# quickwit-oss/quickwit

Hardware: AMD Instinct MI355X
Metric: leaf_search_docs_per_sec (higher is better)
Workload: dtype u32+f32; 1 GPU; 3term_bm25_or_100000000; query=body:w00009 OR body:w00010 OR body:w00011, docs_per_gpu=100000000, splits_per_gpu=1, max_hits=10, parallelism=split-dp1

## Files before the change

include/quickwit_amd.h:

```cpp
#ifndef QUICKWIT_AMD_H
#define QUICKWIT_AMD_H

#include <stddef.h>
#include <stdint.h>

#ifdef __cplusplus
extern "C" {
#endif

typedef struct qw_ctx qw_ctx;

typedef struct qw_buf {
    uint8_t* data;
    size_t len;
} qw_buf;

enum qw_status {
    QW_OK = 0,
    QW_ERR_INVALID_ARGUMENT = -1,
    QW_ERR_INVALID_QUERY = -2,
    QW_ERR_NOT_FOUND = -3,
    QW_ERR_INTERNAL = -4,
    QW_ERR_NO_GPU = -5,
    QW_ERR_BAD_SPLIT = -6,
// ... 5 lines not shown

int32_t qw_ctx_add_split(qw_ctx* ctx, const char* split_id,
                         const uint8_t* data, size_t len);
int32_t qw_ctx_remove_split(qw_ctx* ctx, const char* split_id);

int32_t qw_leaf_search(qw_ctx* ctx, const uint8_t* leaf_search_request_pb,
                       size_t len, qw_buf* response_pb_out);

void qw_buf_free(qw_buf* buf);

int32_t qw_fetch_docs(qw_ctx* ctx, const uint8_t* fetch_docs_request_pb,
                      size_t len, qw_buf* response_pb_out);

int32_t qw_leaf_list_terms(qw_ctx* ctx, const uint8_t* leaf_list_terms_request_pb,
                           size_t len, qw_buf* response_pb_out);

int32_t qw_merge_leaf_responses(const uint8_t* search_request_pb,
                                size_t search_request_len,
                                const uint8_t** response_pbs,
                                const size_t* response_lens, size_t n,
                                qw_buf* merged_out);

int32_t qw_finalize_agg_to_json(const uint8_t* blob, size_t len,
                                const char* agg_request_json,
                                qw_buf* json_out);

int32_t qw_regex_match_terms(const char* regex, size_t regex_len,
                             const uint8_t* term_bytes,
                             const uint32_t* term_offsets, size_t num_terms,
                             uint64_t* match_bitmap_out);

int32_t qw_regex_table_stats(const char* regex, size_t regex_len,
                             uint64_t out[3]);

int32_t qw_regex_resolve(const char* regex, size_t regex_len,
                         int32_t tokenizer_lowercases, qw_buf* resolved_out);

const char* qw_last_error(const qw_ctx* ctx);


int32_t qw_kernel_stats(qw_ctx* ctx, const char* kernel_name,
                        double* total_ms, uint64_t* launches);
void qw_kernel_stats_reset(qw_ctx* ctx);
int32_t qw_ctx_device_sync(qw_ctx* ctx);

int32_t qw_ctx_memory_stats(qw_ctx* ctx, uint64_t* used_bytes,
                            uint64_t* budget_bytes, uint64_t* splits_bytes);

int32_t qw_absence_cache_stats(qw_ctx* ctx, uint64_t* hits, uint64_t* misses,
                               uint64_t* entries);

int32_t qw_topk_stats(qw_ctx* ctx, uint64_t out[4]);

const char* qw_version(void);

#ifdef __cplusplus
}
#endif

#endif
```

quickwit_amd/api.py:

```python
import ctypes
import json
import os

from . import proto

REPO_ROOT = os.path.dirname(os.path.dirname(os.path.abspath(__file__)))


class _Buf(ctypes.Structure):
    _fields_ = [("data", ctypes.POINTER(ctypes.c_uint8)), ("len", ctypes.c_size_t)]


def _bind(lib, syms):
    getattr(lib, syms["create"]).restype = ctypes.c_void_p
    getattr(lib, syms["add_split"]).argtypes = [
        ctypes.c_void_p, ctypes.c_char_p, ctypes.c_char_p, ctypes.c_size_t]
    getattr(lib, syms["leaf_search"]).argtypes = [
        ctypes.c_void_p, ctypes.c_char_p, ctypes.c_size_t, ctypes.POINTER(_Buf)]
    getattr(lib, syms["last_error"]).restype = ctypes.c_char_p
    getattr(lib, syms["last_error"]).argtypes = [ctypes.c_void_p]
    getattr(lib, syms["buf_free"]).argtypes = [ctypes.POINTER(_Buf)]


class _BaseSearcher:
# ... 106 lines not shown
    def leaf_list_terms(self, req: dict) -> dict:
        fn = self._lib.qw_leaf_list_terms
        fn.argtypes = [ctypes.c_void_p, ctypes.c_char_p, ctypes.c_size_t,
                       ctypes.POINTER(_Buf)]
        req_pb = proto.encode("LeafListTermsRequest", req)
        buf = _Buf()
        rc = fn(self._ctx, req_pb, len(req_pb), ctypes.byref(buf))
        if rc != 0:
            raise RuntimeError(f"leaf_list_terms failed ({rc}): {self._err()}")
        out = ctypes.string_at(buf.data, buf.len)
        self._lib.qw_buf_free(ctypes.byref(buf))
        return proto.decode("LeafListTermsResponse", out)

    def kernel_stats(self, name: str):
        fn = self._lib.qw_kernel_stats
        fn.argtypes = [ctypes.c_void_p, ctypes.c_char_p,
                       ctypes.POINTER(ctypes.c_double), ctypes.POINTER(ctypes.c_uint64)]
        ms = ctypes.c_double()
        n = ctypes.c_uint64()
        rc = fn(self._ctx, name.encode(), ctypes.byref(ms), ctypes.byref(n))
        if rc != 0:
            raise KeyError(name)
        return ms.value, n.value

    def kernel_stats_reset(self):
        self._lib.qw_kernel_stats_reset.argtypes = [ctypes.c_void_p]
        self._lib.qw_kernel_stats_reset(self._ctx)

    def memory_stats(self):
        fn = self._lib.qw_ctx_memory_stats
        fn.argtypes = [ctypes.c_void_p] + [ctypes.POINTER(ctypes.c_uint64)] * 3
        u, b, s = ctypes.c_uint64(), ctypes.c_uint64(), ctypes.c_uint64()
        rc = fn(self._ctx, ctypes.byref(u), ctypes.byref(b), ctypes.byref(s))
        if rc != 0:
            raise RuntimeError(f"memory_stats failed: {rc}")
        return u.value, b.value, s.value

    def absence_cache_stats(self):
        fn = self._lib.qw_absence_cache_stats
        fn.argtypes = [ctypes.c_void_p] + [ctypes.POINTER(ctypes.c_uint64)] * 3
        h, m, e = ctypes.c_uint64(), ctypes.c_uint64(), ctypes.c_uint64()
        rc = fn(self._ctx, ctypes.byref(h), ctypes.byref(m), ctypes.byref(e))
        if rc != 0:
            raise RuntimeError(f"absence_cache_stats failed: {rc}")
        return h.value, m.value, e.value

    def topk_stats(self):
        fn = self._lib.qw_topk_stats
        fn.argtypes = [ctypes.c_void_p, ctypes.POINTER(ctypes.c_uint64 * 4)]
        out = (ctypes.c_uint64 * 4)()
        rc = fn(self._ctx, ctypes.byref(out))
        if rc != 0:
            raise RuntimeError(f"topk_stats failed: {rc}")
        return tuple(out)

    def device_sync(self):
        self._lib.qw_ctx_device_sync.argtypes = [ctypes.c_void_p]
        rc = self._lib.qw_ctx_device_sync(self._ctx)
        if rc != 0:
            raise RuntimeError(f"device_sync failed: {self._err()}")


def _product_lib():
    path = os.environ.get("QW_PRODUCT_LIB") or os.path.join(
        REPO_ROOT, "libquickwit_amd.so")
    if not os.path.exists(path):
        raise FileNotFoundError(
            f"{path} not built — run __graft_entry__.build() first")
    lib = ctypes.CDLL(path)
    lib.qw_last_error.restype = ctypes.c_char_p
    lib.qw_last_error.argtypes = [ctypes.c_void_p]
    return lib


def regex_match_terms(regex: str | bytes, terms: list) -> list:
    lib = _product_lib()
    raw = [t.encode() if isinstance(t, str) else bytes(t) for t in terms]
    offsets = (ctypes.c_uint32 * (len(raw) + 1))()
    pos = 0
    for i, t in enumerate(raw):
        offsets[i] = pos
        pos += len(t)
    offsets[len(raw)] = pos
    packed = b"".join(raw)
    words = (ctypes.c_uint64 * max(1, (len(raw) + 63) // 64))()
    rx = regex.encode() if isinstance(regex, str) else bytes(regex)
    fn = lib.qw_regex_match_terms
    fn.argtypes = [ctypes.c_char_p, ctypes.c_size_t, ctypes.c_char_p,
                   ctypes.POINTER(ctypes.c_uint32), ctypes.c_size_t,
                   ctypes.POINTER(ctypes.c_uint64)]
    rc = fn(rx, len(rx), packed, offsets, len(raw), words)
    if rc != 0:
        msg = lib.qw_last_error(None)
        raise ValueError(msg.decode(errors="replace") if msg else f"rc={rc}")
    return [bool((words[i >> 6] >> (i & 63)) & 1) for i in range(len(raw))]


def regex_table_stats(regex: str | bytes) -> tuple:
    lib = _product_lib()
    fn = lib.qw_regex_table_stats
    fn.argtypes = [ctypes.c_char_p, ctypes.c_size_t,
                   ctypes.POINTER(ctypes.c_uint64 * 3)]
    rx = regex.encode() if isinstance(regex, str) else bytes(regex)
    out = (ctypes.c_uint64 * 3)()
    rc = fn(rx, len(rx), ctypes.byref(out))
    if rc != 0:
# ... 58 lines not shown
```

quickwit_amd/csrc/gpu_types.h:

```cpp
#pragma once
#include <cstdint>

namespace qw {

#ifndef QW_TILE_DOCS
#define QW_TILE_DOCS 8192
#endif
constexpr uint32_t TILE_DOCS = QW_TILE_DOCS;
constexpr uint32_t TILE_THREADS = 256;
constexpr uint32_t KTAB_LDS_MAX = 4;
constexpr uint32_t AGG_LDS_BUCKETS = 2048;
constexpr uint32_t TOPK_BINS = 4096;

enum TermRole : uint32_t { ROLE_SHOULD = 0, ROLE_MUST = 1, ROLE_MUST_NOT = 2 };

struct TermDev {
    uint32_t role;
    uint32_t grp;
    uint32_t n_blocks;
    uint64_t skip_off;
    uint64_t payload_off;
    uint64_t norms_off;
    float weight;
    uint32_t ktab_idx;
// ... 68 lines not shown
    uint32_t c_histo;
    uint32_t c_missing;
    double c_interval[4], c_offset[4];
    int64_t c_base[4];
    uint32_t p_si;
    uint64_t p_out;
    int32_t p_k_lo;
    uint32_t p_n_keys;
    uint64_t p_bound_off;
};

struct QueryDev {
    const uint8_t* split;
    const uint8_t* scratch;
    uint8_t* results;
    uint32_t num_docs;
    uint32_t n_tiles;
    uint32_t n_terms;
    uint32_t n_must;
    uint32_t n_must_not;
    uint32_t n_preds;
    uint32_t n_aggs;
    uint32_t msm;
    uint32_t scoring;
    uint32_t match_all;
    uint32_t collect_hits;
    uint32_t sort_asc;
    uint32_t wide_cand;
    uint32_t sort_src;
    uint32_t sort_width;
    uint64_t sort_values_off;
    uint64_t sort_nulls_off;
    uint32_t agg_fast;
    uint32_t agg_nt;
    uint32_t nt_decode;
    uint64_t bitmap_out;
    uint64_t terms_off;
    uint64_t preds_off;
    uint64_t aggs_off;
    uint64_t ktabs_off;
    uint32_t n_ktabs;
    uint32_t _pad_ktab;
    uint64_t norms_stage_off;
    uint64_t tile_counts_off;
    uint64_t cand_count_off;
    uint64_t cand_off;
    uint64_t cand_cap;
    uint64_t hist_off;
    uint32_t prune_k;
    uint32_t gates_off;
};

constexpr uint32_t TOPK_BOUND_OFF = 16;
constexpr uint32_t TOPK_PRUNE_MAX_K = 64;
inline uint32_t* cand_hdr_candidates(uint8_t* hdr) { return (uint32_t*)hdr; }
inline uint32_t* cand_hdr_survivors(uint8_t* hdr) { return (uint32_t*)hdr + 1; }
inline uint32_t* cand_hdr_cursor_band(uint8_t* hdr) { return (uint32_t*)hdr + 2; }

}
```

quickwit_amd/csrc/kernels.hip:

```cpp
#include <hip/hip_runtime.h>

#include "gpu_types.h"

namespace qw {

#pragma pack(push, 1)
struct SkipEntryDev {
    uint32_t first_doc;
    uint32_t last_doc;
    uint32_t word_off;
    uint8_t id_bits;
    uint8_t tf_bits;
    uint16_t count;
};
#pragma pack(pop)

__device__ __forceinline__ uint32_t lane_id() { return threadIdx.x & 63u; }

__device__ __forceinline__ uint64_t extract_bits(const uint32_t* base, uint64_t bitpos,
                                                 uint32_t w) {
    uint64_t word = bitpos >> 5;
    uint32_t sh = uint32_t(bitpos & 31);
    uint64_t v = (uint64_t(base[word]) | (uint64_t(base[word + 1]) << 32)) >> sh;
    return v & ((1ull << w) - 1ull);
// ... 1073 lines not shown
                                               uint32_t* hist) {
    __shared__ uint32_t lh[TOPK_BINS];
    for (uint32_t i = threadIdx.x; i < TOPK_BINS; i += bdim) lh[i] = 0;
    __syncthreads();
    uint32_t n = *n_ptr;
    uint32_t shift = 64 - prefix_bits - 12;
    uint32_t last_bin = 0xFFFFFFFFu, acc = 0;
    for (uint32_t i = blockIdx.x * bdim + threadIdx.x; i < n;
         i += gridDim.x * bdim) {
        uint64_t k = cand[RW * i];
        if (prefix_bits && (k >> (64 - prefix_bits)) != prefix) continue;
        uint32_t b = uint32_t(k >> shift) & (TOPK_BINS - 1);
        if (b == last_bin) ++acc;
        else {
            if (acc) atomicAdd(&lh[last_bin], acc);
            last_bin = b;
            acc = 1;
        }
    }
    if (acc) atomicAdd(&lh[last_bin], acc);
    __syncthreads();
    for (uint32_t i = threadIdx.x; i < TOPK_BINS; i += bdim)
        if (lh[i]) atomicAdd(&hist[i], lh[i]);
}

template <uint32_t RW>
__device__ __forceinline__ void cand_compact_body(uint32_t bdim,
                                                  const uint64_t* cand, uint32_t n,
                                                  uint64_t floor_key,
                                                  uint64_t ceil_key, uint64_t* out,
                                                  uint32_t* out_count,
                                                  uint32_t cap) {
    for (uint32_t i = blockIdx.x * bdim + threadIdx.x; i < n;
         i += gridDim.x * bdim) {
        uint64_t k = cand[RW * i];
        bool take = k >= floor_key && k <= ceil_key;
        uint64_t mask = __ballot(take);
        uint32_t nw = __popcll(mask);
        if (!nw) continue;
        uint32_t leader = __ffsll((unsigned long long)mask) - 1;
        uint32_t base;
        if (lane_id() == leader) base = atomicAdd(out_count, nw);
        base = __shfl(base, leader, 64);
        if (take) {
            uint32_t off = base + __popcll(mask & ((1ull << lane_id()) - 1ull));
            if (off < cap) {
                out[RW * off] = k;
                if (RW == 2) out[2 * off + 1] = cand[2 * i + 1];
            }
        }
    }
}

extern "C" __global__ void k_cand_hist(const uint64_t* cand, const uint32_t* n_ptr,
                                       uint64_t prefix, uint32_t prefix_bits,
                                       uint32_t* hist) {
    cand_hist_body<1>(blockDim.x, cand, n_ptr, prefix, prefix_bits, hist);
}
extern "C" __global__ void k_cand_hist_w(const uint64_t* cand, const uint32_t* n_ptr,
                                         uint64_t prefix, uint32_t prefix_bits,
                                         uint32_t* hist) {
    cand_hist_body<2>(blockDim.x, cand, n_ptr, prefix, prefix_bits, hist);
}
extern "C" __global__ void k_cand_compact(const uint64_t* cand, uint32_t n,
                                          uint64_t floor_key, uint64_t ceil_key,
                                          uint64_t* out, uint32_t* out_count,
                                          uint32_t cap) {
    cand_compact_body<1>(blockDim.x, cand, n, floor_key, ceil_key, out, out_count, cap);
}
extern "C" __global__ void k_cand_compact_w(const uint64_t* cand, uint32_t n,
                                            uint64_t floor_key, uint64_t ceil_key,
                                            uint64_t* out, uint32_t* out_count,
                                            uint32_t cap) {
    cand_compact_body<2>(blockDim.x, cand, n, floor_key, ceil_key, out, out_count, cap);
}

}

namespace qw {

struct PhraseTokDev {
    uint64_t skip_off;
    uint64_t payload_off;
    uint64_t pos_start_off;
    uint64_t positions_off;
    uint32_t n_blocks;
    uint32_t df;
};
constexpr uint32_t PHRASE_MAX_TOKS = 8;
struct PhraseDev {
    uint32_t n_toks;
    uint32_t num_docs;
    PhraseTokDev tok[PHRASE_MAX_TOKS];
};

__device__ __forceinline__ uint32_t phrase_gap(const uint32_t* gw, uint32_t j,
                                               uint32_t w) {
    return uint32_t(extract_bits(gw, uint64_t(j) * w, w));
}

__device__ static uint32_t phrase_doc_at(const uint32_t* payload,
                                         const SkipEntryDev& e, uint32_t j) {
    const uint32_t* gw = payload + e.word_off;
    uint32_t seg = j >> 5;
    uint32_t doc = seg == 0 ? e.first_doc : (gw - 4)[seg];
    for (uint32_t i = seg == 0 ? 1 : seg * 32; i <= j; ++i)
// ... 395 lines not shown
```

quickwit_amd/csrc/product.cpp:

```cpp
#include <hip/hip_runtime.h>
#include <zlib.h>

#include <algorithm>
#include <chrono>
#include <cmath>
#include <cstdint>
#include <cstdlib>
#include <cstring>
#include <list>
#include <map>
#include <memory>
#include <set>
#include <stdexcept>
#include <string>
#include <vector>

#define QW_PHRASE_WINDOW 1
#define QW_REGEX_QUERY 1

#include "../../include/quickwit_amd.h"
#include "fieldnorm.h"
#include "minijson.h"
#include "pb.h"
#include "qagg_format.h"
// ... 213 lines not shown
            } else ++it;
        }
    }
    void clear() {
        for (auto& e : lru) (void)hipFree(e.bm);
        lru.clear();
        idx.clear();
        bytes = 0;
    }
};

}

struct AbsenceCache {
    std::set<std::string> keys;
    uint64_t hits = 0, misses = 0;
    size_t cap = 1 << 20;
    static std::string key(const std::string& split_id, const std::string& f,
                           const std::string& t) {
        std::string k = split_id;
        k += '\0';
        k += f;
        k += '\x1f';
        k += t;
        return k;
    }
    void remove_split(const std::string& split_id) {
        std::string lo = split_id + '\0';
        std::string hi = split_id + '\x01';
        keys.erase(keys.lower_bound(lo), keys.lower_bound(hi));
    }
};

struct qw_ctx {
    int device = 0;
    bool device_ready = false;
    int64_t agg_bucket_limit = 65000;
    std::map<std::string, std::unique_ptr<qw::DeviceSplit>> splits;
    qw::LeafCache leaf_cache;
    qw::HitsetCache hitsets;
    AbsenceCache absence;
    std::string last_error;
    hipStream_t stream = nullptr;
    hipEvent_t ev_start = nullptr, ev_stop = nullptr;
    qw::DevBuf d_scratch, d_results, d_survivors, d_cand2;
    qw::PinnedBuf h_scratch, h_counts, h_surv, h_topk, h_agg;
    std::map<std::string, qw::KernelTimer> timers;
    uint64_t hbm_used = 0;
    uint64_t hbm_budget = 0;
    bool budget_configured = false;
    bool topk_prune = true;
    uint64_t topk_pruned = 0, topk_unpruned = 0;
    uint64_t topk_last_emitted = 0, topk_last_matched = 0;
};

static void qw_check_budget(qw_ctx* ctx, uint64_t need) {
    uint64_t used = ctx->hbm_used + ctx->hitsets.bytes;
    if (ctx->hbm_budget && used + need > ctx->hbm_budget)
        throw std::runtime_error(
            "HBM memory budget exceeded: used " + std::to_string(used) +
            " + need " + std::to_string(need) + " > budget " +
            std::to_string(ctx->hbm_budget) +
            " (search_permit_provider analog; raise hbm_memory_budget or "
            "remove splits)");
}

static void qw_ensure_acct(qw_ctx* ctx, qw::DevBuf& b, size_t n) {
    if (n <= b.cap) return;
    qw_check_budget(ctx, n - b.cap);
    ctx->hbm_used -= b.cap;
    b.ensure(n);
    ctx->hbm_used += b.cap;
}

static uint64_t term_ranges_addr(qw_ctx* ctx, const qw::DeviceSplit& ds,
                                 const qw::TextFieldView* f, int64_t tid,
                                 uint32_t n_tiles, uint32_t num_docs) {
    using namespace qw;
    auto key = std::make_pair((const void*)f, tid);
    auto it = ds.range_cache.find(key);
    if (it != ds.range_cache.end()) return (uint64_t)it->second;
    if (ds.range_cache.size() >= 1024) {
        ctx->hbm_used -= ds.range_cache_bytes;
        ds.free_range_cache();
    }
    size_t bytes = 2ull * n_tiles * 4;
    qw_check_budget(ctx, bytes);
    std::vector<uint32_t> r(2ull * n_tiles);
    const SkipEntry* sk = f->h_skip + f->h_skip_off[tid] / 16;
    uint32_t nb = f->h_n_blocks[tid];
    uint32_t* lo = r.data();
    uint32_t* hi = lo + n_tiles;
    uint32_t b_lo = 0, b_hi = 0;
    for (uint32_t tile = 0; tile < n_tiles; ++tile) {
        uint32_t tlo = tile * TILE_DOCS;
        uint32_t thi = std::min<uint32_t>(tlo + TILE_DOCS, num_docs);
        while (b_lo < nb && sk[b_lo].last_doc < tlo) ++b_lo;
        if (b_hi < b_lo) b_hi = b_lo;
        while (b_hi < nb && sk[b_hi].first_doc < thi) ++b_hi;
        lo[tile] = b_lo;
        hi[tile] = b_hi;
    }
    uint8_t* d = nullptr;
    HIP_CHECK(hipMalloc(&d, bytes));
    HIP_CHECK(hipMemcpy(d, r.data(), bytes, hipMemcpyHostToDevice));
    ctx->hbm_used += bytes;
// ... 1788 lines not shown
    uint32_t n_should = uint32_t(tt.terms.size()) - tt.n_must - tt.n_must_not;
    tl.ns = n_should > 0 || (fq.scoring && !tt.terms.empty());
    tl.nb = tt.n_must > 0 || tt.n_must_not > 0;
    tl.na = do_aggs && !ap.devs.empty();
    tl.grid = n_tiles;
    if (tl.na)
        tl.grid = fq.terms.empty()
                      ? std::min<uint32_t>(
                            {n_tiles, 2048u, std::max<uint32_t>(256u, n_tiles / 8)})
                      : std::min<uint32_t>(n_tiles, 2048u);
    if (tl.na && !ap.devs.empty() && ap.devs[0].kind == AGGD_HISTO &&
        ap.devs[0].lds_slot == 0 && ap.devs[0].int_fast &&
        ap.devs[0].n_sub == 0 && ap.devs[0].nulls_off == 0 &&
        ap.devs.size() <= 2 &&
        (ap.devs.size() < 2 ||
         (ap.devs[1].kind == AGGD_TERMS && ap.devs[1].lds_slot == 1 &&
          ap.devs[1].nulls_off == 0 && ap.devs[1].offsets_off == 0 &&
          ap.devs[1].n_buckets > 0)))
        q.agg_fast = 1;
    if (tl.na && ap.devs.size() == 1 && ap.devs[0].kind == AGGD_TERMS &&
        ap.devs[0].lds_slot == 1 && ap.devs[0].n_sub == 0 &&
        ap.devs[0].nulls_off == 0 && ap.devs[0].offsets_off == 0 &&
        ap.devs[0].n_buckets > 0)
        q.agg_fast = 1;
    static const bool agg_nt = getenv("QW_AGG_NT") != nullptr;
    q.agg_nt = agg_nt ? 1 : 0;
    static const bool nt_decode = getenv("QW_NT_DECODE") != nullptr;
    q.nt_decode = nt_decode ? 1 : 0;
    return tl;
}

static void launch_cand_hist(bool wide, uint32_t grid, hipStream_t stream,
                             const uint64_t* cand, const uint32_t* n_ptr,
                             uint64_t prefix, uint32_t prefix_bits,
                             uint32_t* hist) {
    if (wide)
        hipLaunchKernelGGL(k_cand_hist_w, dim3(grid), dim3(256), 0, stream, cand,
                           n_ptr, prefix, prefix_bits, hist);
    else
        hipLaunchKernelGGL(k_cand_hist, dim3(grid), dim3(256), 0, stream, cand,
                           n_ptr, prefix, prefix_bits, hist);
}
static void launch_cand_compact(bool wide, uint32_t grid, hipStream_t stream,
                                const uint64_t* cand, uint32_t n,
                                uint64_t floor_key, uint64_t ceil_key,
                                uint64_t* out, uint32_t* out_count, uint32_t cap) {
    if (wide)
        hipLaunchKernelGGL(k_cand_compact_w, dim3(grid), dim3(256), 0, stream,
                           cand, n, floor_key, ceil_key, out, out_count, cap);
    else
        hipLaunchKernelGGL(k_cand_compact, dim3(grid), dim3(256), 0, stream, cand,
                           n, floor_key, ceil_key, out, out_count, cap);
}

static uint64_t cursor_ceil_key(const SortPlan& sp, bool fq_scoring) {
    const SortKey& k1 = sp.ck1.key;
    if (sp.wide) {
        if (!k1.has) return 0;
        uint64_t S = k1.key;
        if (sp.specs[0].comp == SortSpec::SCORE) {
            uint32_t kh = f32_sortable_h(float(u64_to_f64(S)));
            S = (uint64_t(kh) << 32) | 0xFFFFFFFFull;
        } else if (sp.specs[0].ff &&
                   sp.specs[0].ff->type == FastFieldView::DATETIME) {
            int64_t ns = u64_to_i64(S);
            int64_t ms = ns / 1000000 - ((ns % 1000000) < 0 ? 1 : 0);
            S = i64_to_u64(ms);
        }
        return sp.order1 == 0 ? ~S : S;
    }
    uint32_t kh = 0;
    if (fq_scoring && k1.has) kh = f32_sortable_h(float(u64_to_f64(k1.key)));
    if (sp.sort_asc()) kh = ~kh;
    return (uint64_t(kh) << 32) | 0xFFFFFFFFull;
}

struct TopkSelector {
    qw_ctx* ctx;
    bool wide, after;
    uint32_t rw;
    uint64_t leaf_max_hits;
    uint64_t* d_cand = nullptr;
    uint32_t* d_n = nullptr;
    uint32_t* d_hist = nullptr;
    uint32_t *d_candidates = nullptr, *d_survivors = nullptr, *d_band = nullptr;
    uint32_t* hist0;
    bool hist0_valid = false;
    uint64_t band_n = 0;
    uint64_t kwant = 0;
    std::vector<uint64_t> top_keys;

    TopkSelector(qw_ctx* c, bool wide_, bool after_, uint64_t leaf_max_hits_)
        : ctx(c), wide(wide_), after(after_), rw(wide_ ? 2 : 1),
          leaf_max_hits(leaf_max_hits_) {
        ctx->h_surv.ensure(TOPK_BINS * 4);
        hist0 = (uint32_t*)ctx->h_surv.p;
    }

    void attach(const ScratchLayout& L) {
        uint8_t* hdr = ctx->d_results.p + L.r_cand_count;
        d_cand = (uint64_t*)(ctx->d_results.p + L.r_cand);
        d_hist = (uint32_t*)(ctx->d_results.p + L.r_hist);
        d_candidates = cand_hdr_candidates(hdr);
        d_survivors = cand_hdr_survivors(hdr);
        d_band = cand_hdr_cursor_band(hdr);
        d_n = d_candidates;
    }

    void enqueue_pass0(uint32_t num_docs) {
        HIP_CHECK(hipMemsetAsync(d_hist, 0, TOPK_BINS * 4, ctx->stream));
        uint32_t hgrid = std::min<uint32_t>(512, (num_docs + 4095) / 4096);
        launch_cand_hist(wide, hgrid, ctx->stream, d_cand, d_candidates, 0ull, 0u,
                         d_hist);
        HIP_CHECK(hipMemcpyAsync(hist0, d_hist, TOPK_BINS * 4,
                                 hipMemcpyDeviceToHost, ctx->stream));
        hist0_valid = true;
    }

    void compact_cursor_band(uint64_t ceil_key) {
        uint32_t cand_n = uint32_t(band_n);
        qw_ensure_acct(ctx, ctx->d_cand2, size_t(cand_n) * 8 * rw + 16);
        HIP_CHECK(hipMemsetAsync(d_band, 0, 4, ctx->stream));
        uint32_t pgrid = std::min<uint32_t>(2048, (cand_n + 255) / 256);
        launch_cand_compact(wide, pgrid, ctx->stream, d_cand, cand_n, 0ull,
                            ceil_key, (uint64_t*)ctx->d_cand2.p, d_band, cand_n);
        uint32_t n2 = 0;
        HIP_CHECK(hipMemcpyAsync(&n2, d_band, 4, hipMemcpyDeviceToHost,
                                 ctx->stream));
        HIP_CHECK(hipStreamSynchronize(ctx->stream));
        d_cand = (uint64_t*)ctx->d_cand2.p;
        d_n = d_band;
        band_n = n2;
    }

    void select(uint64_t Kwant) {
        kwant = Kwant;
        const uint32_t cand_n = uint32_t(band_n);
        uint64_t K = std::min<uint64_t>(Kwant, cand_n);
        uint64_t prefix = 0;
        uint32_t prefix_bits = 0;
        uint64_t survivors = cand_n, above = 0, Krem = K;
        uint64_t floor_key = 0;
        std::vector<uint32_t> hist(TOPK_BINS);
        HIP_CHECK(hipEventRecord(ctx->ev_start, ctx->stream));
        while (true) {
            if (survivors <= std::max<uint64_t>(4 * K, 16384) || prefix_bits >= 48) {
                if (prefix_bits == 0) floor_key = 0;
                break;
            }
            if (prefix_bits == 0 && hist0_valid) {
                memcpy(hist.data(), hist0,
                       TOPK_BINS * 4);
            } else {
                HIP_CHECK(hipMemsetAsync(d_hist, 0, TOPK_BINS * 4, ctx->stream));
                uint32_t hgrid = std::min<uint32_t>(512, (cand_n + 4095) / 4096);
                launch_cand_hist(wide, hgrid, ctx->stream, d_cand, d_n, prefix,
                                 prefix_bits, d_hist);
                HIP_CHECK(hipMemcpyAsync(hist.data(), d_hist, TOPK_BINS * 4,
                                         hipMemcpyDeviceToHost, ctx->stream));
                HIP_CHECK(hipStreamSynchronize(ctx->stream));
            }
            uint64_t cum = 0;
            int b = TOPK_BINS - 1;
            for (; b >= 0; --b) {
                if (cum + hist[b] >= Krem) break;
                cum += hist[b];
            }
            if (b < 0) b = 0;
            uint32_t shift = 64 - prefix_bits - 12;
            floor_key = (prefix_bits ? (prefix << (64 - prefix_bits)) : 0) |
                        (uint64_t(uint32_t(b)) << shift);
            above += cum;
            survivors = above + hist[b];
            Krem = Krem - cum;
            prefix = (prefix << 12) | uint64_t(uint32_t(b));
            prefix_bits += 12;
        }
        qw_ensure_acct(ctx, ctx->d_survivors, survivors * 8 * rw + 16);
        HIP_CHECK(hipMemsetAsync(d_survivors, 0, 4, ctx->stream));
        uint32_t cgrid = std::min<uint32_t>(2048, (cand_n + 255) / 256);
        launch_cand_compact(wide, cgrid, ctx->stream, d_cand, cand_n, floor_key,
                            ~0ull, (uint64_t*)ctx->d_survivors.p, d_survivors,
                            uint32_t(survivors));
        top_keys.resize(survivors * rw);
        ctx->h_topk.ensure(survivors * 8 * rw + 16);
        HIP_CHECK(hipMemcpyAsync(ctx->h_topk.p, ctx->d_survivors.p,
                                 survivors * 8 * rw, hipMemcpyDeviceToHost,
                                 ctx->stream));
        HIP_CHECK(hipEventRecord(ctx->ev_stop, ctx->stream));
        HIP_CHECK(hipStreamSynchronize(ctx->stream));
        memcpy(top_keys.data(), ctx->h_topk.p, survivors * 8 * rw);
        float tms = 0;
        HIP_CHECK(hipEventElapsedTime(&tms, ctx->ev_start, ctx->ev_stop));
        record_kernel_time(ctx, "topk_select", tms);
        if (!wide) {
            std::sort(top_keys.begin(), top_keys.end(), std::greater<uint64_t>());
            if (top_keys.size() > K && !after) top_keys.resize(K);
        }
    }

    bool grow(size_t n_hits) {
        if (!after || band_n == 0 ||
            n_hits >= std::min<uint64_t>(leaf_max_hits, band_n) || kwant >= band_n)
            return false;
        select(std::min<uint64_t>(band_n, kwant * 8));
        return true;
    }
};

struct TileRun {
    uint64_t matched = 0;
    uint32_t cand_n = 0;
};

static void enqueue_uploads(qw_ctx* ctx, const ScratchLayout& L,
                            const AggPlan& ap, bool do_aggs) {
    HIP_CHECK(hipMemcpyAsync(ctx->d_scratch.p, ctx->h_scratch.p, L.scratch_bytes,
                             hipMemcpyHostToDevice, ctx->stream));
    HIP_CHECK(hipMemsetAsync(ctx->d_results.p, 0, L.r_agg, ctx->stream));
    if (do_aggs && ap.out_bytes)
        HIP_CHECK(hipMemcpyAsync(ctx->d_results.p + L.r_agg, ap.init.data(),
                                 ap.out_bytes, hipMemcpyHostToDevice, ctx->stream));
}

static TileRun run_leaf_tile(qw_ctx* ctx, const SplitView& sv,
                             const TileLaunch& tl, const ScratchLayout& L,
                             const AggPlan& ap, bool collect, bool do_aggs,
                             TopkSelector& sel, StageTimer& timer) {
    const uint32_t n_tiles = tl.q.n_tiles;
    HIP_CHECK(hipEventRecord(ctx->ev_start, ctx->stream));
    launch_leaf_tile(tl.ns, tl.nb, tl.na, collect, dim3(tl.grid), ctx->stream,
                     tl.q, 0u, n_tiles, 1u);
    HIP_CHECK(hipEventRecord(ctx->ev_stop, ctx->stream));
    HIP_CHECK(hipGetLastError());
    if (collect && !sel.after) sel.enqueue_pass0(sv.num_docs);

    ctx->h_counts.ensure(size_t(n_tiles) * 4 + 64);
    uint32_t* tile_counts = (uint32_t*)ctx->h_counts.p;
    uint32_t* pc = (uint32_t*)(ctx->h_counts.p + size_t(n_tiles) * 4);
    HIP_CHECK(hipMemcpyAsync(tile_counts, ctx->d_results.p + L.r_tile_counts,
                             size_t(n_tiles) * 4, hipMemcpyDeviceToHost,
                             ctx->stream));
    if (collect)
        HIP_CHECK(hipMemcpyAsync(pc, ctx->d_results.p + L.r_cand_count, 4,
                                 hipMemcpyDeviceToHost, ctx->stream));
    if (do_aggs && ap.out_bytes) {
        ctx->h_agg.ensure(ap.out_bytes + 64);
        HIP_CHECK(hipMemcpyAsync(ctx->h_agg.p, ctx->d_results.p + L.r_agg,
                                 ap.out_bytes, hipMemcpyDeviceToHost,
                                 ctx->stream));
    }
    HIP_CHECK(hipStreamSynchronize(ctx->stream));
    TileRun run;
    run.cand_n = collect ? *pc : 0;
    timer.mark("main+pass0+sync");
    float ms = 0;
    HIP_CHECK(hipEventElapsedTime(&ms, ctx->ev_start, ctx->ev_stop));
    record_kernel_time(ctx, tl.kname, ms);
    for (uint32_t i = 0; i < n_tiles; ++i) run.matched += tile_counts[i];
    if (collect) {
        ++(tl.q.prune_k ? ctx->topk_pruned : ctx->topk_unpruned);
        ctx->topk_last_emitted = run.cand_n;
        ctx->topk_last_matched = run.matched;
    }
    return run;
}

static pb::PartialHit make_hit(const SplitView& sv, const SortPlan& sp,
                               uint32_t doc, float score) {
    pb::PartialHit h;
    h.split_id = sv.split_id;
    h.segment_ord = sv.segment_ord;
    h.doc_id = doc;
    if (!sp.specs.empty()) h.sort_value = sort_value_of(sp.specs[0], doc, score);
    if (sp.specs.size() > 1) h.sort_value2 = sort_value_of(sp.specs[1], doc, score);
    return h;
}

static void build_hits(std::vector<pb::PartialHit>& hits, const SplitView& sv,
                       const SortPlan& sp, bool fq_scoring, TopkSelector& sel,
                       uint64_t leaf_max_hits, bool trivial_hits) {
    if (trivial_hits) {
        uint64_t k = std::min<uint64_t>(leaf_max_hits, sv.num_docs);
        for (uint64_t i = 0; i < k; ++i) {
            uint32_t doc = sp.order1 == 1 ? uint32_t(sv.num_docs - 1 - i)
                                          : uint32_t(i);
            hits.push_back(make_hit(sv, sp, doc, 0.f));
        }
        return;
    }
    const std::vector<uint64_t>& top_keys = sel.top_keys;
    do {
        hits.clear();
        hits.reserve(top_keys.size() / (sp.wide ? 2 : 1));
        if (sp.wide) {
            size_t n = top_keys.size() / 2;
            for (size_t i = 0; i < n; ++i) {
                uint64_t aux = top_keys[2 * i + 1];
                uint32_t doc = uint32_t(aux);
                float score = 0.f;
                if (fq_scoring) {
                    uint32_t b = uint32_t(aux >> 32);
                    memcpy(&score, &b, 4);
                }
                hits.push_back(make_hit(sv, sp, doc, score));
            }
// ... 217 lines not shown
}

static SplitResult search_split_gpu(qw_ctx* ctx, const DeviceSplit& ds,
                                    const pb::SearchRequest& req, const Schema& schema) {
    SplitResult out;
    StageTimer timer;
    const SplitView& sv = ds.view;
    ctx->hitsets.begin_query();

    PlanNode plan = leaf_plan(ctx, sv, req, schema);
    SortPlan sp = make_sort_plan(sv, req);
    GateBitmaps gate_tmp(ctx);
    FlatQuery fq = flatten_or_bitmap(ctx, ds, plan, schema, sp.scoring, gate_tmp);
    out.absent_required = fq.absent_required;
    const uint64_t leaf_max_hits = req.max_hits + req.start_offset;
    const bool do_aggs = req.aggregation_request.has_value();

    if (fq.match_none || sv.num_docs == 0) {
        if (do_aggs) {
            empty_agg_shapes(*req.aggregation_request, out.aggs);
            out.has_aggs = true;
        }
        out.micros = timer.micros();
        return out;
    }

    const uint32_t n_tiles = (sv.num_docs + TILE_DOCS - 1) / TILE_DOCS;
    const bool pure_match_all =
        fq.match_all && fq.preds.empty() && fq.terms.empty();
    const bool trivial_hits = pure_match_all && sp.specs.empty() && !sp.after;
    const bool collect = leaf_max_hits > 0 && !trivial_hits && !fq.match_none;
    const bool need_kernel = !pure_match_all || do_aggs || collect;

    TermTables tt = build_term_tables(sv, fq);
    ScratchLayout L = layout_results_head(n_tiles);
    AggPlan ap;
    if (do_aggs)
        ap = plan_aggs(sv, *req.aggregation_request, ctx->agg_bucket_limit,
                       L.r_agg);
    layout_finish(L, tt, fq, ap, collect ? sv.num_docs : 0, sp.wide);
    eager_pred_flags(sv, fq);
    timer.mark("plan");
    ctx->h_scratch.ensure(L.scratch_bytes);
    for (size_t i = 0; i < fq.terms.size(); ++i) {
        const FlatQuery::FTerm& t = fq.terms[i];
        tt.terms[i].ranges_addr =
            term_ranges_addr(ctx, ds, t.f, t.tid, n_tiles, sv.num_docs);
    }
    timer.mark("ranges");
    assemble_scratch(ctx->h_scratch.p, L, tt, fq, ap);
    timer.mark("assembly");

    uint64_t matched = sv.num_docs;
    TopkSelector sel(ctx, sp.wide, sp.after != nullptr, leaf_max_hits);
    if (need_kernel) {
        qw_ensure_acct(ctx, ctx->d_scratch, L.scratch_bytes);
        qw_ensure_acct(ctx, ctx->d_results, L.results_bytes);
        sel.attach(L);
        enqueue_uploads(ctx, L, ap, do_aggs);
        TileLaunch tl = fill_query_dev(ctx, ds, fq, sp, tt, ap, L, collect,
                                       do_aggs, leaf_max_hits, n_tiles);
        TileRun run = run_leaf_tile(ctx, sv, tl, L, ap, collect, do_aggs, sel, timer);
        matched = run.matched;
        if (collect && run.cand_n > 0) {
            sel.band_n = run.cand_n;
            if (sp.after) sel.compact_cursor_band(cursor_ceil_key(sp, fq.scoring));
            if (sel.band_n > 0) {
                sel.select(std::min<uint64_t>(
                    leaf_max_hits + (sp.after ? 1024 : 0), sel.band_n));
                timer.mark("topk_select");
            }
        }
    }
    if (pure_match_all) matched = sv.num_docs;
    out.num_hits = matched;

    if (leaf_max_hits > 0)
        build_hits(out.hits, sv, sp, fq.scoring, sel, leaf_max_hits, trivial_hits);
    timer.mark("build_hits");

    if (do_aggs) {
        ctx->h_agg.ensure(ap.out_bytes + 64);
        decode_aggs(ap, L.r_agg, ctx->h_agg.p, matched, out.aggs);
        out.has_aggs = true;
    }
    timer.mark("aggs_assembly");

    out.micros = timer.micros();
    return out;
}

static SplitResult search_device_split(qw_ctx* ctx, const DeviceSplit& ds,
                                       const pb::SearchRequest& req,
                                       const Schema& schema) {
    using namespace qw;
    std::vector<const DeviceSplit*> segs;
    if (ds.segs.empty()) segs.push_back(&ds);
    else
        for (auto& sp : ds.segs) segs.push_back(sp.get());
    SplitResult out;
    std::map<std::pair<std::string, std::string>, size_t> absent;
    for (const DeviceSplit* seg : segs) {
        SplitResult r = search_split_gpu(ctx, *seg, req, schema);
        out.num_hits += r.num_hits;
        for (auto& h : r.hits) out.hits.push_back(std::move(h));
        if (r.has_aggs) {
            if (!out.has_aggs) {
                out.aggs = std::move(r.aggs);
                out.has_aggs = true;
            } else out.aggs.merge(r.aggs);
        }
        out.micros += r.micros;
        for (auto& ab : r.absent_required) absent[ab]++;
    }
    const std::string& sid = segs[0]->view.split_id;
    for (auto& kv : absent)
        if (kv.second == segs.size() &&
            ctx->absence.keys.size() < ctx->absence.cap)
            ctx->absence.keys.insert(
                AbsenceCache::key(sid, kv.first.first, kv.first.second));
    uint64_t leaf_max = req.max_hits + req.start_offset;
    if (segs.size() > 1 && leaf_max > 0 && !out.hits.empty()) {
        int order1, order2;
        request_sort_orders(req, &order1, &order2);
        size_t k = std::min<uint64_t>(leaf_max, out.hits.size());
        std::partial_sort(out.hits.begin(), out.hits.begin() + k,
                          out.hits.end(),
                          [&](const pb::PartialHit& a, const pb::PartialHit& b) {
                              return hit_before(a, b, order1, order2);
                          });
        out.hits.resize(k);
    }
    return out;
}

static int64_t split_ts_start(const pb::SplitIdAndFooterOffsets& s) {
// ... 65 lines not shown
    if (r.start_timestamp || r.end_timestamp) return false;
    try {
        mj::ValuePtr v = mj::parse(r.query_ast);
        const mj::Value* t = v->get("type");
        return t && t->kind == mj::Value::STR && t->s == "match_all";
    } catch (...) {
        return false;
    }
}

static void disable_search_request_hits(pb::SearchRequest& r) {
    r.max_hits = 0;
    r.start_offset = 0;
    r.sort_fields.clear();
    r.search_after.reset();
}

}

static thread_local std::string g_tls_error;

static void set_err(qw_ctx* ctx, const std::string& msg) {
    if (ctx) ctx->last_error = msg;
    else g_tls_error = msg;
}

static void fill_buf(qw_buf* out, const std::string& s) {
    out->data = (uint8_t*)malloc(s.size() ? s.size() : 1);
    memcpy(out->data, s.data(), s.size());
    out->len = s.size();
}

extern "C" {

const char* qw_version(void) { return "quickwit_amd 0.1 gfx950"; }

qw_ctx* qw_ctx_create(const char* config_json) {
    auto* ctx = new qw_ctx();
    try {
        if (config_json && *config_json) {
            mj::ValuePtr cfg = mj::parse(config_json);
            if (const mj::Value* d = cfg->get("device")) ctx->device = int(d->as_i64());
            if (const mj::Value* b = cfg->get("aggregation_bucket_limit"))
                ctx->agg_bucket_limit = b->as_i64();
            if (const mj::Value* c = cfg->get("partial_request_cache_capacity"))
                ctx->leaf_cache.capacity = size_t(c->as_i64());
            if (const mj::Value* mb = cfg->get("hbm_memory_budget")) {
                ctx->hbm_budget = uint64_t(mb->as_i64());
                ctx->budget_configured = true;
            }
            if (const mj::Value* tp = cfg->get("topk_prune"))
                ctx->topk_prune = tp->kind == mj::Value::BOOL ? tp->b
                                                              : tp->as_i64() != 0;
        }
        return ctx;
    } catch (const std::exception& e) {
        g_tls_error = e.what();
        delete ctx;
        return nullptr;
    }
}

void qw_ctx_free(qw_ctx* ctx) {
    if (!ctx) return;
    if (ctx->device_ready) {
        (void)hipSetDevice(ctx->device);
        for (auto& kv : ctx->splits) {
            kv.second->free_range_cache();
            for (auto& sg : kv.second->segs) sg->free_range_cache();
            if (kv.second->d_image) (void)hipFree(kv.second->d_image);
        }
        ctx->hitsets.clear();
        if (ctx->ev_start) (void)hipEventDestroy(ctx->ev_start);
        if (ctx->ev_stop) (void)hipEventDestroy(ctx->ev_stop);
        if (ctx->stream) (void)hipStreamDestroy(ctx->stream);
    }
    delete ctx;
}

const char* qw_last_error(const qw_ctx* ctx) {
    return ctx ? ctx->last_error.c_str() : g_tls_error.c_str();
}

int32_t qw_ctx_add_split(qw_ctx* ctx, const char* split_id, const uint8_t* data,
                         size_t len) {
    using namespace qw;
    try {
        ctx_ensure_device(ctx);
    } catch (const std::exception& e) {
        set_err(ctx, e.what());
        return QW_ERR_NO_GPU;
    }
    try {
        auto ds = std::make_unique<DeviceSplit>();
        ds->host.assign(data, data + len);
        if (len >= 88 && memcmp(data, "QWAMDSP2", 8) == 0) {
            if (memcmp(data + len - 8, "QWA1FOOT", 8) != 0)
                throw std::runtime_error("bad QWA2 footer");
            uint64_t moff, mlen;
            memcpy(&moff, data + len - 24, 8);
            memcpy(&mlen, data + len - 16, 8);
            if (moff + mlen > len) throw std::runtime_error("bad QWA2 footer");
            mj::ValuePtr meta = mj::parse((const char*)data + moff, mlen);
            uint32_t ord = 0;
            for (auto& sgv : meta->at("segments")->arr) {
                uint64_t off = uint64_t(sgv->at("off")->as_i64());
// ... 619 lines not shown

int32_t qw_kernel_stats(qw_ctx* ctx, const char* kernel_name, double* total_ms,
                        uint64_t* launches) {
    auto it = ctx->timers.find(kernel_name);
    if (it == ctx->timers.end()) {
        static const char* known[] = {"union_bm25", "range_filter", "column_agg",
                                      "topk_select", "k_dict_dfa_match",
                                      "k_terms_union_bitmap"};
        bool ok = false;
        for (const char* k : known) ok |= kernel_name == std::string(k);
        if (!ok) return QW_ERR_NOT_FOUND;
        *total_ms = 0;
        *launches = 0;
        return QW_OK;
    }
    *total_ms = it->second.total_ms;
    *launches = it->second.launches;
    return QW_OK;
}

void qw_kernel_stats_reset(qw_ctx* ctx) { ctx->timers.clear(); }

int32_t qw_ctx_memory_stats(qw_ctx* ctx, uint64_t* used_bytes,
                            uint64_t* budget_bytes, uint64_t* splits_bytes) {
    if (!ctx) return QW_ERR_INVALID_ARGUMENT;
    if (used_bytes) *used_bytes = ctx->hbm_used + ctx->hitsets.bytes;
    if (budget_bytes) *budget_bytes = ctx->hbm_budget;
    if (splits_bytes) {
        uint64_t sb = 0;
        for (auto& kv : ctx->splits) sb += kv.second->len + 64;
        *splits_bytes = sb;
    }
    return QW_OK;
}

int32_t qw_absence_cache_stats(qw_ctx* ctx, uint64_t* hits, uint64_t* misses,
                               uint64_t* entries) {
    if (!ctx) return QW_ERR_INVALID_ARGUMENT;
    if (hits) *hits = ctx->absence.hits;
    if (misses) *misses = ctx->absence.misses;
    if (entries) *entries = uint64_t(ctx->absence.keys.size());
    return QW_OK;
}

int32_t qw_topk_stats(qw_ctx* ctx, uint64_t out[4]) {
    if (!ctx || !out) return QW_ERR_INVALID_ARGUMENT;
    out[0] = ctx->topk_pruned;
    out[1] = ctx->topk_unpruned;
    out[2] = ctx->topk_last_emitted;
    out[3] = ctx->topk_last_matched;
    return QW_OK;
}

int32_t qw_ctx_device_sync(qw_ctx* ctx) {
    try {
        ctx_ensure_device(ctx);
        HIP_CHECK(hipDeviceSynchronize());
        return QW_OK;
    } catch (const std::exception& e) {
        set_err(ctx, e.what());
        return QW_ERR_NO_GPU;
    }
}

}
```

Measured before the change: 165.6 billion docs/s.

## Fuse top-K threshold pick and compaction on device to need one host sync

Adds a device kernel that scans the pass-0 score histogram to choose a floor bucket and then compacts the surviving candidates in the same launch. The host reads the results header, histogram, aggregations and the first block of survivors in one transfer followed by a single stream sync, so the separate histogram-download and select round trips go away. If too many candidates survive, it falls back to the old multi-pass refine. The cost is a redundant per-block histogram scan, a larger contiguous copy of the results head, and a second sync when survivors exceed the inline buffer.

After: 176.5 billion docs/s, median of 6. 6.6% higher.

```diff
diff --git a/include/quickwit_amd.h b/include/quickwit_amd.h
--- a/include/quickwit_amd.h
+++ b/include/quickwit_amd.h
@@ -81,6 +81,8 @@
 
 int32_t qw_topk_stats(qw_ctx* ctx, uint64_t out[4]);
 
+int32_t qw_topk_onesync_stats(qw_ctx* ctx, uint64_t out[4]);
+
 const char* qw_version(void);
 
 #ifdef __cplusplus
diff --git a/quickwit_amd/api.py b/quickwit_amd/api.py
--- a/quickwit_amd/api.py
+++ b/quickwit_amd/api.py
@@ -182,6 +182,15 @@
         rc = fn(self._ctx, ctypes.byref(out))
         if rc != 0:
             raise RuntimeError(f"topk_stats failed: {rc}")
+        return tuple(out)
+
+    def topk_onesync_stats(self):
+        fn = self._lib.qw_topk_onesync_stats
+        fn.argtypes = [ctypes.c_void_p, ctypes.POINTER(ctypes.c_uint64 * 4)]
+        out = (ctypes.c_uint64 * 4)()
+        rc = fn(self._ctx, ctypes.byref(out))
+        if rc != 0:
+            raise RuntimeError(f"topk_onesync_stats failed: {rc}")
         return tuple(out)
 
     def device_sync(self):
diff --git a/quickwit_amd/csrc/gpu_types.h b/quickwit_amd/csrc/gpu_types.h
--- a/quickwit_amd/csrc/gpu_types.h
+++ b/quickwit_amd/csrc/gpu_types.h
@@ -144,7 +144,12 @@
 };
 
 constexpr uint32_t TOPK_BOUND_OFF = 16;
+constexpr uint32_t TOPK_PICK_COUNT_OFF = 24;
+constexpr uint32_t TOPK_PICK_REFINE_OFF = 28;
+constexpr uint32_t TOPK_PICK_FLOOR_OFF = 32;
 constexpr uint32_t TOPK_PRUNE_MAX_K = 64;
+constexpr uint32_t TOPK_REFINE_MIN = 16384;
+constexpr uint32_t TOPK_INLINE_SURVIVORS = 4096;
 inline uint32_t* cand_hdr_candidates(uint8_t* hdr) { return (uint32_t*)hdr; }
 inline uint32_t* cand_hdr_survivors(uint8_t* hdr) { return (uint32_t*)hdr + 1; }
 inline uint32_t* cand_hdr_cursor_band(uint8_t* hdr) { return (uint32_t*)hdr + 2; }
diff --git a/quickwit_amd/csrc/kernels.hip b/quickwit_amd/csrc/kernels.hip
--- a/quickwit_amd/csrc/kernels.hip
+++ b/quickwit_amd/csrc/kernels.hip
@@ -1149,6 +1149,109 @@
     }
 }
 
+struct TopkPick {
+    uint64_t floor_key;
+    uint32_t survivors;
+    uint32_t refine;
+};
+constexpr uint32_t TOPK_PICK_THREADS = 256;
+constexpr uint32_t TOPK_PICK_BINS = TOPK_BINS / TOPK_PICK_THREADS;
+static_assert(TOPK_PICK_BINS == 16, "topk_pick loads its bins as four uint4");
+
+__device__ __forceinline__ TopkPick topk_pick(const uint32_t* hist, uint32_t n,
+                                              uint32_t kwant) {
+    TopkPick p;
+    const uint32_t K = kwant < n ? kwant : n;
+    const uint64_t k4 = 4ull * K;
+    const uint64_t T = k4 > TOPK_REFINE_MIN ? k4 : TOPK_REFINE_MIN;
+    p.floor_key = 0;
+    p.survivors = n;
+    p.refine = 0;
+    if (n <= T) return p;
+
+    __shared__ uint32_t scan[TOPK_PICK_THREADS];
+    __shared__ uint32_t found[3];
+    const uint32_t t = threadIdx.x;
+    const uint32_t lo = TOPK_BINS - TOPK_PICK_BINS * (t + 1);
+    uint32_t h[TOPK_PICK_BINS];
+    const uint4* src = (const uint4*)(hist + lo);
+#pragma unroll
+    for (uint32_t j = 0; j < TOPK_PICK_BINS / 4; ++j) {
+        uint4 v = src[j];
+        h[4 * j] = v.x;
+        h[4 * j + 1] = v.y;
+        h[4 * j + 2] = v.z;
+        h[4 * j + 3] = v.w;
+    }
+    uint32_t own = 0;
+#pragma unroll
+    for (uint32_t j = 0; j < TOPK_PICK_BINS; ++j) own += h[j];
+    scan[t] = own;
+    if (t == 0) found[0] = 0xFFFFFFFFu;
+    __syncthreads();
+    for (uint32_t off = 1; off < TOPK_PICK_THREADS; off <<= 1) {
+        uint32_t v = t >= off ? scan[t - off] : 0;
+        __syncthreads();
+        scan[t] += v;
+        __syncthreads();
+    }
+    const uint32_t incl = scan[t], excl = incl - own;
+    if (excl < K && incl >= K) {
+        uint32_t cum = excl, b = 0, hb = 0;
+        bool done = false;
+#pragma unroll
+        for (int j = int(TOPK_PICK_BINS) - 1; j >= 0; --j) {
+            if (done) continue;
+            if (cum + h[j] >= K) {
+                done = true;
+                b = lo + uint32_t(j);
+                hb = h[j];
+            } else cum += h[j];
+        }
+        found[0] = b;
+        found[1] = cum;
+        found[2] = hb;
+    }
+    __syncthreads();
+    if (found[0] == 0xFFFFFFFFu) {
+        p.refine = 1;
+        return p;
+    }
+    p.floor_key = uint64_t(found[0]) << (64 - 12);
+    p.survivors = found[1] + found[2];
+    p.refine = p.survivors > T ? 1 : 0;
+    return p;
+}
+
+template <uint32_t RW>
+__device__ __forceinline__ void cand_pick_compact_body(
+    uint32_t bdim, const uint64_t* cand, uint32_t cand_cap, uint32_t* hdr,
+    const uint32_t* hist, uint32_t kwant, uint64_t* out, uint32_t cap) {
+    uint32_t n = hdr[0];
+    if (n > cand_cap) n = cand_cap;
+    TopkPick p = topk_pick(hist, n, kwant);
+    if (blockIdx.x == 0 && threadIdx.x == 0) {
+        hdr[TOPK_PICK_COUNT_OFF / 4] = p.survivors;
+        hdr[TOPK_PICK_REFINE_OFF / 4] = p.refine;
+        *(uint64_t*)(hdr + TOPK_PICK_FLOOR_OFF / 4) = p.floor_key;
+    }
+    if (p.refine) return;
+    cand_compact_body<RW>(bdim, cand, n, p.floor_key, ~0ull, out, hdr + 1, cap);
+}
+
+extern "C" __global__ void __launch_bounds__(TOPK_PICK_THREADS)
+k_cand_pick_compact(const uint64_t* cand, uint32_t cand_cap, uint32_t* hdr,
+                    const uint32_t* hist, uint32_t kwant, uint64_t* out,
+                    uint32_t cap) {
+    cand_pick_compact_body<1>(blockDim.x, cand, cand_cap, hdr, hist, kwant, out, cap);
+}
+extern "C" __global__ void __launch_bounds__(TOPK_PICK_THREADS)
+k_cand_pick_compact_w(const uint64_t* cand, uint32_t cand_cap, uint32_t* hdr,
+                      const uint32_t* hist, uint32_t kwant, uint64_t* out,
+                      uint32_t cap) {
+    cand_pick_compact_body<2>(blockDim.x, cand, cand_cap, hdr, hist, kwant, out, cap);
+}
+
 extern "C" __global__ void k_cand_hist(const uint64_t* cand, const uint32_t* n_ptr,
                                        uint64_t prefix, uint32_t prefix_bits,
                                        uint32_t* hist) {
diff --git a/quickwit_amd/csrc/product.cpp b/quickwit_amd/csrc/product.cpp
--- a/quickwit_amd/csrc/product.cpp
+++ b/quickwit_amd/csrc/product.cpp
@@ -289,6 +289,9 @@
     bool topk_prune = true;
     uint64_t topk_pruned = 0, topk_unpruned = 0;
     uint64_t topk_last_emitted = 0, topk_last_matched = 0;
+    bool topk_onesync = true;
+    uint64_t topk_onesync_calls = 0, topk_onesync_fallbacks = 0;
+    uint64_t topk_onesync_last_survivors = 0, topk_onesync_last_tail = 0;
 };
 
 static void qw_check_budget(qw_ctx* ctx, uint64_t need) {
@@ -2183,6 +2186,19 @@
         hipLaunchKernelGGL(k_cand_compact, dim3(grid), dim3(256), 0, stream, cand,
                            n, floor_key, ceil_key, out, out_count, cap);
 }
+static void launch_cand_pick_compact(bool wide, uint32_t grid, hipStream_t stream,
+                                     const uint64_t* cand, uint32_t cand_cap,
+                                     uint32_t* hdr, const uint32_t* hist,
+                                     uint32_t kwant, uint64_t* out, uint32_t cap) {
+    if (wide)
+        hipLaunchKernelGGL(k_cand_pick_compact_w, dim3(grid),
+                           dim3(TOPK_PICK_THREADS), 0, stream, cand, cand_cap, hdr,
+                           hist, kwant, out, cap);
+    else
+        hipLaunchKernelGGL(k_cand_pick_compact, dim3(grid),
+                           dim3(TOPK_PICK_THREADS), 0, stream, cand, cand_cap, hdr,
+                           hist, kwant, out, cap);
+}
 
 static uint64_t cursor_ceil_key(const SortPlan& sp, bool fq_scoring) {
     const SortKey& k1 = sp.ck1.key;
@@ -2220,6 +2236,11 @@
     uint64_t band_n = 0;
     uint64_t kwant = 0;
     std::vector<uint64_t> top_keys;
+    uint32_t* d_hdr = nullptr;
+    uint32_t cand_cap = 0;
+    uint32_t surv_cap = 0;
+    bool onesync = false;
+    uint32_t picked_survivors = 0;
 
     TopkSelector(qw_ctx* c, bool wide_, bool after_, uint64_t leaf_max_hits_)
         : ctx(c), wide(wide_), after(after_), rw(wide_ ? 2 : 1),
@@ -2236,16 +2257,104 @@
         d_survivors = cand_hdr_survivors(hdr);
         d_band = cand_hdr_cursor_band(hdr);
         d_n = d_candidates;
-    }
-
-    void enqueue_pass0(uint32_t num_docs) {
-        HIP_CHECK(hipMemsetAsync(d_hist, 0, TOPK_BINS * 4, ctx->stream));
+        d_hdr = (uint32_t*)hdr;
+        cand_cap = uint32_t(L.cand_cap);
+    }
+
+    void enqueue_pass0(uint32_t num_docs, bool prezeroed = false) {
+        if (!prezeroed)
+            HIP_CHECK(hipMemsetAsync(d_hist, 0, TOPK_BINS * 4, ctx->stream));
         uint32_t hgrid = std::min<uint32_t>(512, (num_docs + 4095) / 4096);
         launch_cand_hist(wide, hgrid, ctx->stream, d_cand, d_candidates, 0ull, 0u,
                          d_hist);
+    }
+
+    void download_pass0() {
         HIP_CHECK(hipMemcpyAsync(hist0, d_hist, TOPK_BINS * 4,
                                  hipMemcpyDeviceToHost, ctx->stream));
         hist0_valid = true;
+    }
+
+    bool onesync_wanted(bool collect) const {
+        return collect && !after && ctx->topk_onesync;
+    }
+
+    void reserve_onesync(uint32_t num_docs) {
+        uint64_t k = std::min<uint64_t>(leaf_max_hits, num_docs);
+        uint64_t t = std::min<uint64_t>(std::max<uint64_t>(4 * k, TOPK_REFINE_MIN),
+                                        num_docs);
+        surv_cap = uint32_t(std::max<uint64_t>(t, TOPK_INLINE_SURVIVORS));
+        qw_ensure_acct(ctx, ctx->d_survivors, size_t(surv_cap) * 8 * rw + 16);
+        ctx->h_topk.ensure(size_t(TOPK_INLINE_SURVIVORS) * 8 * rw);
+    }
+
+    void enqueue_onesync(uint32_t num_docs, bool few) {
+        enqueue_pass0(num_docs, true);
+        uint32_t cgrid = few ? 256u
+                             : std::min<uint32_t>(2048, (num_docs + 1023) / 1024);
+        uint32_t kw = uint32_t(std::min<uint64_t>(leaf_max_hits, 0xFFFFFFFFull));
+        launch_cand_pick_compact(wide, cgrid, ctx->stream, d_cand, cand_cap, d_hdr,
+                                 d_hist, kw, (uint64_t*)ctx->d_survivors.p,
+                                 surv_cap);
+        HIP_CHECK(hipMemcpyAsync(ctx->h_topk.p, ctx->d_survivors.p,
+                                 size_t(TOPK_INLINE_SURVIVORS) * 8 * rw,
+                                 hipMemcpyDeviceToHost, ctx->stream));
+        onesync = true;
+    }
+
+    void onesync_arrived(const uint8_t* hdr, const uint8_t* hist) {
+        uint32_t refine, compacted;
+        memcpy(&picked_survivors, hdr + TOPK_PICK_COUNT_OFF, 4);
+        memcpy(&refine, hdr + TOPK_PICK_REFINE_OFF, 4);
+        memcpy(&compacted, hdr + 4, 4);
+        hist0 = (uint32_t*)hist;
+        hist0_valid = true;
+        if (refine) {
+            onesync = false;
+            ++ctx->topk_onesync_fallbacks;
+            return;
+        }
+        if (compacted != picked_survivors || picked_survivors > surv_cap)
+            throw std::runtime_error(
+                "top-K one-sync selection: histogram and compaction disagree (" +
+                std::to_string(picked_survivors) + " vs " +
+                std::to_string(compacted) + ")");
+        ++ctx->topk_onesync_calls;
+        ctx->topk_onesync_last_survivors = picked_survivors;
+        ctx->topk_onesync_last_tail = picked_survivors > TOPK_INLINE_SURVIVORS;
+    }
+
+    void take_onesync(uint64_t K) {
+        const size_t rec = size_t(8) * rw;
+        const size_t n = picked_survivors;
+        const size_t inl = std::min<size_t>(n, TOPK_INLINE_SURVIVORS);
+        top_keys.resize(n * rw);
+        memcpy(top_keys.data(), ctx->h_topk.p, inl * rec);
+        if (n > inl) {
+            ctx->h_topk.ensure((n - inl) * rec);
+            HIP_CHECK(hipEventRecord(ctx->ev_start, ctx->stream));
+            HIP_CHECK(hipMemcpyAsync(ctx->h_topk.p, ctx->d_survivors.p + inl * rec,
+                                     (n - inl) * rec, hipMemcpyDeviceToHost,
+                                     ctx->stream));
+            HIP_CHECK(hipEventRecord(ctx->ev_stop, ctx->stream));
+            HIP_CHECK(hipStreamSynchronize(ctx->stream));
+            memcpy(top_keys.data() + inl * rw, ctx->h_topk.p, (n - inl) * rec);
+            float tms = 0;
+            HIP_CHECK(hipEventElapsedTime(&tms, ctx->ev_start, ctx->ev_stop));
+            record_kernel_time(ctx, "topk_select", tms);
+        }
+        sort_truncate(K);
+    }
+
+    void sort_truncate(uint64_t K) {
+        if (wide) return;
+        const bool cut = top_keys.size() > K && !after;
+        if (cut && K <= top_keys.size() / 8)
+            std::partial_sort(top_keys.begin(), top_keys.begin() + K,
+                              top_keys.end(), std::greater<uint64_t>());
+        else
+            std::sort(top_keys.begin(), top_keys.end(), std::greater<uint64_t>());
+        if (cut) top_keys.resize(K);
     }
 
     void compact_cursor_band(uint64_t ceil_key) {
@@ -2268,6 +2377,11 @@
         kwant = Kwant;
         const uint32_t cand_n = uint32_t(band_n);
         uint64_t K = std::min<uint64_t>(Kwant, cand_n);
+        if (onesync) {
+            onesync = false;
+            take_onesync(K);
+            return;
+        }
         uint64_t prefix = 0;
         uint32_t prefix_bits = 0;
         uint64_t survivors = cand_n, above = 0, Krem = K;
@@ -2324,10 +2438,7 @@
         float tms = 0;
         HIP_CHECK(hipEventElapsedTime(&tms, ctx->ev_start, ctx->ev_stop));
         record_kernel_time(ctx, "topk_select", tms);
-        if (!wide) {
-            std::sort(top_keys.begin(), top_keys.end(), std::greater<uint64_t>());
-            if (top_keys.size() > K && !after) top_keys.resize(K);
-        }
+        sort_truncate(K);
     }
 
     bool grow(size_t n_hits) {
@@ -2342,6 +2453,7 @@
 struct TileRun {
     uint64_t matched = 0;
     uint32_t cand_n = 0;
+    const uint8_t* agg_host = nullptr;
 };
 
 static void enqueue_uploads(qw_ctx* ctx, const ScratchLayout& L,
@@ -2364,25 +2476,45 @@
                      tl.q, 0u, n_tiles, 1u);
     HIP_CHECK(hipEventRecord(ctx->ev_stop, ctx->stream));
     HIP_CHECK(hipGetLastError());
-    if (collect && !sel.after) sel.enqueue_pass0(sv.num_docs);
-
-    ctx->h_counts.ensure(size_t(n_tiles) * 4 + 64);
-    uint32_t* tile_counts = (uint32_t*)ctx->h_counts.p;
-    uint32_t* pc = (uint32_t*)(ctx->h_counts.p + size_t(n_tiles) * 4);
-    HIP_CHECK(hipMemcpyAsync(tile_counts, ctx->d_results.p + L.r_tile_counts,
-                             size_t(n_tiles) * 4, hipMemcpyDeviceToHost,
-                             ctx->stream));
-    if (collect)
-        HIP_CHECK(hipMemcpyAsync(pc, ctx->d_results.p + L.r_cand_count, 4,
+    const bool agg_out = do_aggs && ap.out_bytes;
+    TileRun run;
+    uint32_t* tile_counts;
+    uint32_t* pc;
+    if (sel.onesync_wanted(collect)) {
+        sel.enqueue_onesync(sv.num_docs, tl.q.prune_k != 0);
+        const size_t head = agg_out ? L.r_agg + ap.out_bytes : L.r_agg;
+        ctx->h_counts.ensure(head + 64);
+        HIP_CHECK(hipMemcpyAsync(ctx->h_counts.p, ctx->d_results.p, head,
                                  hipMemcpyDeviceToHost, ctx->stream));
-    if (do_aggs && ap.out_bytes) {
-        ctx->h_agg.ensure(ap.out_bytes + 64);
-        HIP_CHECK(hipMemcpyAsync(ctx->h_agg.p, ctx->d_results.p + L.r_agg,
-                                 ap.out_bytes, hipMemcpyDeviceToHost,
+        HIP_CHECK(hipStreamSynchronize(ctx->stream));
+        tile_counts = (uint32_t*)(ctx->h_counts.p + L.r_tile_counts);
+        pc = (uint32_t*)(ctx->h_counts.p + L.r_cand_count);
+        run.agg_host = ctx->h_counts.p + L.r_agg;
+        sel.onesync_arrived(ctx->h_counts.p + L.r_cand_count,
+                            ctx->h_counts.p + L.r_hist);
+    } else {
+        if (collect && !sel.after) {
+            sel.enqueue_pass0(sv.num_docs);
+            sel.download_pass0();
+        }
+        ctx->h_counts.ensure(size_t(n_tiles) * 4 + 64);
+        tile_counts = (uint32_t*)ctx->h_counts.p;
+        pc = (uint32_t*)(ctx->h_counts.p + size_t(n_tiles) * 4);
+        HIP_CHECK(hipMemcpyAsync(tile_counts, ctx->d_results.p + L.r_tile_counts,
+                                 size_t(n_tiles) * 4, hipMemcpyDeviceToHost,
                                  ctx->stream));
-    }
-    HIP_CHECK(hipStreamSynchronize(ctx->stream));
-    TileRun run;
+        if (collect)
+            HIP_CHECK(hipMemcpyAsync(pc, ctx->d_results.p + L.r_cand_count, 4,
+                                     hipMemcpyDeviceToHost, ctx->stream));
+        if (do_aggs) ctx->h_agg.ensure(ap.out_bytes + 64);
+        if (agg_out) {
+            HIP_CHECK(hipMemcpyAsync(ctx->h_agg.p, ctx->d_results.p + L.r_agg,
+                                     ap.out_bytes, hipMemcpyDeviceToHost,
+                                     ctx->stream));
+        }
+        HIP_CHECK(hipStreamSynchronize(ctx->stream));
+        run.agg_host = ctx->h_agg.p;
+    }
     run.cand_n = collect ? *pc : 0;
     timer.mark("main+pass0+sync");
     float ms = 0;
@@ -2706,16 +2838,19 @@
     timer.mark("assembly");
 
     uint64_t matched = sv.num_docs;
+    const uint8_t* agg_host = nullptr;
     TopkSelector sel(ctx, sp.wide, sp.after != nullptr, leaf_max_hits);
     if (need_kernel) {
         qw_ensure_acct(ctx, ctx->d_scratch, L.scratch_bytes);
         qw_ensure_acct(ctx, ctx->d_results, L.results_bytes);
         sel.attach(L);
+        if (sel.onesync_wanted(collect)) sel.reserve_onesync(sv.num_docs);
         enqueue_uploads(ctx, L, ap, do_aggs);
         TileLaunch tl = fill_query_dev(ctx, ds, fq, sp, tt, ap, L, collect,
                                        do_aggs, leaf_max_hits, n_tiles);
         TileRun run = run_leaf_tile(ctx, sv, tl, L, ap, collect, do_aggs, sel, timer);
         matched = run.matched;
+        agg_host = run.agg_host;
         if (collect && run.cand_n > 0) {
             sel.band_n = run.cand_n;
             if (sp.after) sel.compact_cursor_band(cursor_ceil_key(sp, fq.scoring));
@@ -2734,8 +2869,7 @@
     timer.mark("build_hits");
 
     if (do_aggs) {
-        ctx->h_agg.ensure(ap.out_bytes + 64);
-        decode_aggs(ap, L.r_agg, ctx->h_agg.p, matched, out.aggs);
+        decode_aggs(ap, L.r_agg, agg_host, matched, out.aggs);
         out.has_aggs = true;
     }
     timer.mark("aggs_assembly");
@@ -2907,6 +3041,9 @@
             if (const mj::Value* tp = cfg->get("topk_prune"))
                 ctx->topk_prune = tp->kind == mj::Value::BOOL ? tp->b
                                                               : tp->as_i64() != 0;
+            if (const mj::Value* os = cfg->get("topk_onesync"))
+                ctx->topk_onesync = os->kind == mj::Value::BOOL ? os->b
+                                                                : os->as_i64() != 0;
         }
         return ctx;
     } catch (const std::exception& e) {
@@ -3632,6 +3769,15 @@
     return QW_OK;
 }
 
+int32_t qw_topk_onesync_stats(qw_ctx* ctx, uint64_t out[4]) {
+    if (!ctx || !out) return QW_ERR_INVALID_ARGUMENT;
+    out[0] = ctx->topk_onesync_calls;
+    out[1] = ctx->topk_onesync_fallbacks;
+    out[2] = ctx->topk_onesync_last_survivors;
+    out[3] = ctx->topk_onesync_last_tail;
+    return QW_OK;
+}
+
 int32_t qw_ctx_device_sync(qw_ctx* ctx) {
     try {
         ctx_ensure_device(ctx);
```
